# jwheo12/RustRayTrace

Measured on AMD Instinct MI355X. Metric: Mrays/sec + wall-clock for 1920×1080×512spp RTOW final scene, higher is better.
Workload: dtype f32; 1 GPU; C2 RTOW final scene (gpu/mod.rs generator, seed 0x5EED1234), 1920x1080x512spp, max_depth 100, 486 spheres; spp=512, max_depth=100, parallelism=whole frame on 1 GPU (the band split with one rank), no gather

## Files before the change

### include/rrt_hip.h

```cpp
#ifndef RRT_HIP_H
#define RRT_HIP_H

#include <stddef.h>
#include <stdint.h>

#ifdef __cplusplus
extern "C" {
#endif

#define RRT_ABI_VERSION 11u


typedef struct RrtCamera {
    float origin[4];
    float pixel00[4];
    float pixel_delta_u[4];
    float pixel_delta_v[4];
    float u[4];
    float v[4];
    float background[4];
    float params_f[4];
    uint32_t params_u[4];
} RrtCamera;

// ... 478 lines not shown
int32_t rrt_testing_launch_plan(const RrtLaunchPlanQuery *query, RrtLaunchPlan *plan);

int32_t rrt_testing_recip_check(uint64_t *mismatches);

int32_t rrt_testing_trig32_check(double *out);

int32_t rrt_testing_sqrt64_check(uint64_t *out);

enum RrtDeviceOp {
    RRT_OP_SIN = 0,
    RRT_OP_COS = 1,
    RRT_OP_LOG = 2,
    RRT_OP_ACOS = 3,
    RRT_OP_ATAN2 = 4,
    RRT_OP_DIV_A = 5,
    RRT_OP_DIV_CONST = 6,
    RRT_OP_FLOOR_I32 = 7,
    RRT_OP_CHECKER = 8,
    RRT_OP_PERLIN = 9,
    RRT_OP_VEC = 10,
    RRT_OP_QUAD = 11,
    RRT_OP_SPHERE = 12,
    RRT_OP_LIGHTS_PDF = 13,
    RRT_OP_LIGHTS_RANDOM = 14
};
int32_t rrt_testing_device_ops(uint32_t op, uint32_t n, const void *in, void *out, const void *aux);

int32_t rrt_testing_div_check(const float *a_values, uint32_t n_a, uint64_t *out);

enum RrtDeviceOp64 {
    RRT_OP_ACOS64 = 0,
    RRT_OP_ATAN2_64 = 1,
    RRT_OP_DIV_A64 = 2,
    RRT_OP_DIV_CONST64 = 3,
    RRT_OP_SQRT64 = 4,
    RRT_OP_AS_I32 = 5,
    RRT_OP_ATT64 = 6,
    RRT_OP_VEC64 = 7,
    RRT_OP_TEXEL64 = 8,
    RRT_OP_SPHERE64 = 9,
    RRT_OP_QUAD64 = 10,
    RRT_OP_CHECKER64 = 11
};
int32_t rrt_testing_device_ops64(uint32_t op, uint32_t n, const void *in, void *out, const void *aux);

#ifdef __cplusplus
}
// ... 3 lines not shown
```

### rustraytrace_amd/_lib.py

```python
from __future__ import annotations

import ctypes
import os
from ctypes import POINTER, c_char_p, c_double, c_float, c_int32, c_size_t, c_uint8, c_uint32, c_uint64, c_void_p

import numpy as np

PKG_DIR = os.path.dirname(os.path.abspath(__file__))
LIB_PATH = os.environ.get("RRT_LIB_PATH") or os.path.join(PKG_DIR, "librrt_hip.so")

CAMERA_DTYPE = np.dtype(
    [
        ("origin", "<f4", 4),
        ("pixel00", "<f4", 4),
        ("pixel_delta_u", "<f4", 4),
        ("pixel_delta_v", "<f4", 4),
        ("u", "<f4", 4),
        ("v", "<f4", 4),
        ("background", "<f4", 4),
        ("params_f", "<f4", 4),
        ("params_u", "<u4", 4),
    ]
)
SPHERE_DTYPE = np.dtype([("center_radius", "<f4", 4), ("material_index", "<u4"), ("_pad", "<u4", 3)])
# ... 129 lines not shown

class RrtSceneBuildStats(ctypes.Structure):
    _fields_ = [("builder", c_uint64), ("launches", c_uint64), ("blocking_reads", c_uint64), ("form", c_uint64),
                ("shape_attempts", c_uint64)]


BUILDERS = {"binned": 0, "lbvh": 1}


class RrtTreeCost(ctypes.Structure):
    _fields_ = [("sah", c_double), ("sah_at_build", c_double), ("refits_since_build", c_uint64)]


def refit_form(form: int) -> None:
    check(load().rrt_testing_refit_form(int(form)))

def lbvh_form(form: int) -> None:
    check(load().rrt_testing_lbvh_form(int(form)))

DEVICE_OPS = {
    "SIN": (0, 1, 1), "COS": (1, 1, 1), "LOG": (2, 1, 1), "ACOS": (3, 1, 1), "ATAN2": (4, 2, 1),
    "DIV_A": (5, 2, 4), "DIV_CONST": (6, 1, 4), "FLOOR_I32": (7, 1, 1), "CHECKER": (8, 4, 1),
    "PERLIN": (9, 3, 8), "VEC": (10, 9, 13), "QUAD": (11, 9, 2), "SPHERE": (12, 11, 13),
    "LIGHTS_PDF": (13, 6, 1), "LIGHTS_RANDOM": (14, 6, 4),
}

DEVICE_OPS64 = {
    "ACOS64": (0, 1, 1), "ATAN2_64": (1, 2, 1), "DIV_A64": (2, 2, 3), "DIV_CONST64": (3, 1, 4), "SQRT64": (4, 1, 1),
    "AS_I32": (5, 1, 1), "ATT64": (6, 2, 4), "VEC64": (7, 9, 11), "TEXEL64": (8, 5, 6), "SPHERE64": (9, 11, 6),
    "QUAD64": (10, 9, 2), "CHECKER64": (11, 4, 1),
}


class RrtTexture(ctypes.Structure):
    _fields_ = [("rgb8", POINTER(c_uint8)), ("width", c_int32), ("height", c_int32)]


PERLIN_DTYPE = np.dtype([("randvec", "<f4", (256, 4)), ("perm_x", "<u2", 256), ("perm_y", "<u2", 256),
                         ("perm_z", "<u2", 256), ("_pad", "<u2", 256)])


QUAD_DTYPE = np.dtype([("q", "<f4", 4), ("u", "<f4", 4), ("v", "<f4", 4), ("material_index", "<u4"),
                       ("_pad", "<u4", 3)])


LIGHT_DTYPE = np.dtype([("kind", "<u4"), ("_pad", "<u4", 3), ("a", "<f4", 4), ("u", "<f4", 4), ("v", "<f4", 4)])

# ... 326 lines not shown
```

### rustraytrace_amd/csrc/rrt_kernel.hip

```cpp
#include "rrt_internal.h"
#include "../../include/rrt_hip.h"

#include <algorithm>
#include <cstddef>
#include <cstdio>
#include <cstdlib>
#include <type_traits>

namespace rrt {
namespace {

#ifndef RRT_PHASE_TIMING
#define RRT_PHASE_TIMING 0
#endif
#ifndef RRT_DEBUG_NOREJECT
#define RRT_DEBUG_NOREJECT 0
#endif
#ifndef RRT_DEBUG_EXTRA_NODE_LOAD
#define RRT_DEBUG_EXTRA_NODE_LOAD 0
#endif
#ifndef RRT_PRIO_REFILL
#define RRT_PRIO_REFILL 2
#endif
#ifndef RRT_PRIO_NODE
// ... 160 lines not shown
__device__ __forceinline__ bool box_hit_ordered(float nx, float fx, float ny, float fy, float nz, float fz, V3 inv,
                                                V3 oi, float tmin, float tmax, float &tnear) {
    const float x0 = __builtin_fmaf(nx, inv.x, -oi.x), x1 = __builtin_fmaf(fx, inv.x, -oi.x);
    const float y0 = __builtin_fmaf(ny, inv.y, -oi.y), y1 = __builtin_fmaf(fy, inv.y, -oi.y);
    const float z0 = __builtin_fmaf(nz, inv.z, -oi.z), z1 = __builtin_fmaf(fz, inv.z, -oi.z);
    const float nr = __builtin_fmaxf(__builtin_fmaxf(x0, y0), __builtin_fmaxf(z0, tmin));
    const float fr = min_f32_raw(__builtin_fminf(__builtin_fminf(x1, y1), z1), tmax);
    tnear = nr;
    return nr < fr;
}


struct RayK {
    V3 inv;
    V3 oi;
    float a;
    float ra;
    uint32_t ox, oy, oz;
};

__device__ __forceinline__ float clamp_inv(float v) { return __builtin_fmaxf(__builtin_fminf(v, 0x1.0p64f), -0x1.0p64f); }
__device__ __forceinline__ float clamped_slope(float s) {
    return __builtin_fabsf(s) < 0x1.0p-126f ? __builtin_copysignf(0x1.0p64f, s) : clamp_inv(recip_rn(s));
}

#ifndef RRT_F16_ORDERED_MAX_CLASS
#define RRT_F16_ORDERED_MAX_CLASS 3
#endif
#ifndef RRT_B1U_WAVES
#define RRT_B1U_WAVES 8
#endif
#ifndef RRT_B1U_BLOCK
#define RRT_B1U_BLOCK 1024
#endif
#ifndef RRT_B1D_WAVES
#define RRT_B1D_WAVES 8
#endif
#ifndef RRT_B2_NF_WAVES
#define RRT_B2_NF_WAVES 6
#endif
#ifndef RRT_B2_MEDIA_GLOBAL_WAVES
#define RRT_B2_MEDIA_GLOBAL_WAVES 0
#endif
__device__ __forceinline__ float refine_ra(float a) {
    const float r0 = __builtin_amdgcn_rcpf(a);
    const float e = __builtin_fmaf(-a, r0, 1.0f);
    return (a >= 0x1.0p-64f && a <= 0x1.0p64f) ? __builtin_fmaf(e, r0, r0) : 0.0f;
}
template <bool kLdsNodes = true, bool kHoldRa = true>
__device__ __forceinline__ RayK ray_consts(V3 o, V3 d) {
    RayK r;
    r.inv = v3(clamped_slope(d.x), clamped_slope(d.y), clamped_slope(d.z));
    r.oi = v3(o.x * r.inv.x, o.y * r.inv.y, o.z * r.inv.z);
    if (kLdsNodes) {
        r.ox = r.inv.x < 0.0f ? 4u : 0u;
        r.oy = r.inv.y < 0.0f ? 16u : 12u;
        r.oz = r.inv.z < 0.0f ? 28u : 24u;
    } else {
        r.ox = (r.inv.x < 0.0f ? 16u : 0u) | (r.inv.y < 0.0f ? 16u << 5 : 0u) | (r.inv.z < 0.0f ? 16u << 10 : 0u);
        r.oy = r.oz = 0u;
    }
    r.a = dot(d, d);
    r.ra = kHoldRa ? refine_ra(r.a) : 0.0f;
    return r;
}

__device__ __forceinline__ float div_by_a(float n, const RayK &rk) {
    const float q0 = n * rk.ra;
    const float m = __builtin_fabsf(q0);
    const bool outside = !(m >= 0x1.0p-30f && m < __builtin_inff());
    const float e0 = __builtin_fmaf(-rk.a, q0, n);
    const float q1 = __builtin_fmaf(e0, rk.ra, q0);
    const float e1 = __builtin_fmaf(-rk.a, q1, n);
    float q = __builtin_fmaf(e1, rk.ra, q1);
    if (__ballot(outside) != 0) {
        float nn = n;
        asm volatile("" : "+v"(nn));
        if (outside) q = nn / rk.a;
    }
    return q;
}

constexpr int kBook1Untextured = -1;
constexpr int kBook1Diffuse = -2;
template <int kBook2>
struct Prims {
    const float4 *cr;
    const float4 *mo;
    float time;
    const GQuad *qd;
    const GMedium *md;
    uint32_t n_quads;
    uint64_t seg;
    const GPerlin *perlin;
    static constexpr bool kHasQuads = kBook2 >= 2;
    static constexpr bool kHasMedia = kBook2 >= 3;
// ... 187 lines not shown
    if constexpr (RRT_PHASE_TIMING == 3) cnt.d2 += 1;
    const float sq = sqrt_rn_disc(disc);
    float root = div_by_a(h - sq, rk);
    uint64_t lt = __ballot(root < closest);
    asm volatile("" : "+v"(root));
    const bool below = !(0.001f < root);
    if (__builtin_expect(__ballot(below) != 0, 0)) {
        float hh = h;
        asm volatile("" : "+v"(hh));
        if (below) root = div_by_a(hh + sq, rk);
        lt = __ballot(0.001f < root) & __ballot(root < closest);
    }
    const bool accept = __builtin_amdgcn_inverse_ballot_w64(lt);
    closest = accept ? root : closest;
    hit_prim = accept ? i : hit_prim;
}

template <bool kCount, class PR>
__device__ __forceinline__ void test_range(const PR &prim_cr, int first, int count, V3 o, V3 d, const RayK &rk,
                                           int skip, float &closest, int &hit_prim, Counters &cnt) {
    if (kCount) cnt.spheres += (uint32_t)count;
    const bool trim = (uint32_t)(skip - first) < (uint32_t)count;
    const int n = count - (trim ? 1 : 0);
    const int gap = trim ? skip : 0x7fffffff;
    for (int k = 0; k < n; ++k) {
        const int i = first + k + (first + k >= gap ? 1 : 0);
        if constexpr (RRT_PHASE_TIMING == 3) {
            cnt.d0 += wave_slot();
            cnt.d1 += 1;
        }
        const float4 cr = prim_cr.cr[i];
        float4 m = cr;
        if constexpr (!PR::kR2) m = prim_cr.mo[i];
        test_prim(prim_cr, cr, m, i, o, d, rk, closest, hit_prim, cnt);
    }
}


struct Trav {
    float closest;
    int hit_prim;
    int node;
    uint32_t sp;
};

__device__ __forceinline__ void trav_begin(Trav &t, int root, uint32_t sp0) {
    t.closest = __builtin_inff();
    t.hit_prim = -1;
    t.node = root;
// ... 135 lines not shown
    cswap(0, 2);
    cswap(1, 3);
    cswap(1, 2);
    const float kInf = __builtin_inff();
    if (key[3] < kInf) { stack.store(t.sp, idx[3]); ++t.sp; }
    if (key[2] < kInf) { stack.store(t.sp, idx[2]); ++t.sp; }
    if (key[1] < kInf) { stack.store(t.sp, idx[1]); ++t.sp; }
    if (key[0] < kInf) {
        t.node = idx[0];
        return false;
    }
    if (t.sp == 0) {
        t.node = -1;
        return true;
    }
    --t.sp;
    t.node = stack.load(t.sp);
    return false;
}

struct PathState {
    V3 o, d, T;
    RngState rng;
    uint32_t k;
    float time;
    int skip;
};

__device__ __forceinline__ int exit_skip(bool is_quad, bool is_medium, bool front, V3 dir, V3 nrm, int prim) {
    if (is_medium) return -1;
    if (is_quad) return prim;
    return ((dot(dir, nrm) > 0.0f) == front) ? prim : -1;
}

template <bool kStrat>
__device__ __forceinline__ void camera_ray(const KParams &P, uint32_t x, uint32_t y, uint32_t s, PathState &ps,
                                           Counters &cnt) {
    const auto &C = *kernarg_params();
    float ox, oy;
    if constexpr (kStrat) {
        const uint32_t sj = fast_div(s, P.fd_sqrt_spp), si = s - sj * P.sqrt_spp;
        ox = (((float)si + rnd(ps.rng)) * P.recip_sqrt_spp) - 0.5f;
        oy = (((float)sj + rnd(ps.rng)) * P.recip_sqrt_spp) - 0.5f;
    } else {
        ox = __builtin_fmaf((float)(rng_next(ps.rng) >> 8), 0x1.0p-24f, -0.5f);
        oy = __builtin_fmaf((float)(rng_next(ps.rng) >> 8), 0x1.0p-24f, -0.5f);
    }
    const float fi = (float)x + ox;
    const float fj = (float)y + oy;
    const V3 sample = v3(C.p00[0] + C.du[0] * fi + C.dv[0] * fj,
                         C.p00[1] + C.du[1] * fi + C.dv[1] * fj,
                         C.p00[2] + C.du[2] * fi + C.dv[2] * fj);
    V3 origin = v3(C.center[0], C.center[1], C.center[2]);
    if (C.defocus_radius > 0.0f) {
        float px, py;
        for (;;) {
            if constexpr (RRT_PHASE_TIMING == 7) cnt.d2 += wave_slot();
            px = rnd_pm1(ps.rng);
            py = rnd_pm1(ps.rng);
            if (__builtin_fmaf(py, py, px * px) < 1.0f) break;
        }
        origin = v3(C.center[0] + C.disk_u[0] * px + C.disk_v[0] * py,
                    C.center[1] + C.disk_u[1] * px + C.disk_v[1] * py,
                    C.center[2] + C.disk_u[2] * px + C.disk_v[2] * py);
    }
    ps.time = 0.0f;
    if (C.flags & 0x1u) ps.time = rnd(ps.rng);
    ps.skip = -1;
    ps.o = origin;
    ps.d = sub(sample, origin);
    ps.T = v3(1.0f, 1.0f, 1.0f);
    ps.k = 0;
}

__device__ __forceinline__ RngState path_rng(const KParams &P, uint32_t x, uint32_t y, uint32_t s) {
    const uint64_t key = pixel_key(P, x, y);
    return rng_seed(splitmix64(key + s), key);
}

__device__ __forceinline__ float rrt_sinf(float xx) {
    float x = xx;
    float sign = 1.0f;
    if (x < 0.0f) { sign = -1.0f; x = -x; }
    if (x > 16777215.0f) return 0.0f;
    if (!(x == x)) return xx;
    int j = (int)(1.27323954473516f * x);
    float y = (float)j;
    if (j & 1) { j += 1; y += 1.0f; }
    j &= 7;
    if (j > 3) { sign = -sign; j -= 4; }
    if (x > 8192.0f) x = x - y * 0.7853981633974483096f;
    else x = ((x - y * 0.78515625f) - y * 2.4187564849853515625e-4f) - y * 3.77489497744594108e-8f;
    const float z = x * x;
    if (j == 1 || j == 2) {
        y = ((2.443315711809948e-5f * z - 1.388731625493765e-3f) * z + 4.166664568298827e-2f) * z * z;
// ... 126 lines not shown
        cnt.d0 += wave_slot();
        cnt.d1 += 1;
    }
    if constexpr (RRT_PHASE_TIMING == 9) cnt.d2 += wave_slot();
    if (prim < 0) {
        if constexpr (RRT_PHASE_TIMING == 6) {
            cnt.d1 += wave_slot();
            cnt.d2 += 1;
        }
        V3 bg;
        if (P.bg_mode == 1u) {
            bg = v3(P.background[0], P.background[1], P.background[2]);
        } else {
            const V3 ud = unit(ps.d);
            const float a = 0.5f * (ud.y + 1.0f);
            bg = v3((1.0f - a) * 1.0f + a * 0.5f, (1.0f - a) * 1.0f + a * 0.7f, (1.0f - a) * 1.0f + a * 1.0f);
        }
        sum = add(sum, mul(ps.T, bg));
        return true;
    }
    float4 qn;
    const float4 cr = prims.at(prim, qn);
    const V3 p = v3(__builtin_fmaf(ps.d.x, t, ps.o.x), __builtin_fmaf(ps.d.y, t, ps.o.y), __builtin_fmaf(ps.d.z, t, ps.o.z));
    V3 outward;
    bool is_quad = false, is_medium = false;
    if (PR::kHasQuads && cr.w < 0.0f) {
        const int j = (int)(-cr.w) - 1;
        if (PR::kHasMedia && j >= (int)prims.n_quads) {
            is_medium = true;
            outward = v3(1.0f, 0.0f, 0.0f);
        } else {
            is_quad = true;
            outward = v3(qn.x, qn.y, qn.z);
        }
    } else {
        const float inv_r = PR::kR2 ? __int_as_float(mtl[prim].b.w) : qn.w;
        outward = v3((p.x - cr.x) * inv_r, (p.y - cr.y) * inv_r, (p.z - cr.z) * inv_r);
    }
    const bool front = dot(ps.d, outward) < 0.0f;
    const V3 nrm = front ? outward : v3(-outward.x, -outward.y, -outward.z);
    const GMaterial m = mtl[prim];
    const int kind = m.b.x;
    V3 att;
    V3 dir;
    if (kind == 4) {
        sum = add(sum, mul(ps.T, v3(m.a.x, m.a.y, m.a.z)));
// ... 12 lines not shown
#define RRT_DEBUG_TEXEL_FIXED 0
#endif
            const float theta = RRT_DEBUG_TEXEL_FIXED ? 1.0f + outward.y * 0x1.0p-30f : rrt_acosf(-outward.y);
            const float phi = RRT_DEBUG_TEXEL_FIXED ? 2.0f + outward.x * 0x1.0p-30f : rrt_atan2f(-outward.z, outward.x) + kPi;
            att = texel(P, m.b.z, div_by_const(phi, 2.0f * kPi), div_by_const(theta, kPi));
        } else if (kBook2 > 0 && kind == 5) {
            att = checker_even(m.a.w, p) ? v3(m.a.x, m.a.y, m.a.z)
                                         : v3(__int_as_float(m.b.y), __int_as_float(m.b.z), __int_as_float(m.b.w));
        } else if (kBook2 > 0 && kNoise && kind == 6) {
            if constexpr (RRT_PHASE_TIMING == 9) {
                cnt.d0 += wave_slot();
                cnt.d1 += 1;
            }
            const float g = noise_at(P, prims.perlin, m.b.z, m.a.w, p);
            att = v3(g, g, g);
        } else {
            att = v3(m.a.x, m.a.y, m.a.z);
        }
    } else if (kind == 1) {
        if constexpr (RRT_PHASE_TIMING == 5) cnt.d2 += wave_slot();
        if constexpr (RRT_PHASE_TIMING == 6) cnt.d0 += 1;
        const V3 refl = unit(reflect(ps.d, nrm));
        dir = add(refl, muls(r, m.a.w));
        if (!(dot(dir, nrm) > 0.0f)) return true;
        att = v3(m.a.x, m.a.y, m.a.z);
    } else {
        if constexpr (RRT_PHASE_TIMING == 5) {
            cnt.d0 += wave_slot();
            cnt.d1 += 1;
        }
        float ri, r0;
        dielectric_ri_r0(m, front, ri, r0);
        const V3 ud = unit(ps.d);
        float c = -dot(ud, nrm);
        c = (c < 1.0f) ? c : 1.0f;
        const float sn = sqrt_rn_big(1.0f - c * c);
        const bool cannot = ri * sn > 1.0f;
        if (cannot || reflectance_r0(c, r0) > rnd(ps.rng)) dir = reflect(ud, nrm);
        else dir = refract(ud, nrm, ri);
        att = v3(1.0f, 1.0f, 1.0f);
    }
    if (ps.k >= 5u) {
        float pr = att.x;
        if (att.y > pr) pr = att.y;
        if (att.z > pr) pr = att.z;
        if (pr < 0.05f) pr = 0.05f;
        if (pr > 0.95f) pr = 0.95f;
        if (rnd(ps.rng) > pr) return true;
        float inv_pr;
        if (kBook2 == kBook1Untextured) inv_pr = kind == 2 ? 1.0f / 0.95f : __int_as_float(m.b.y);
        else inv_pr = recip_rn(pr);
        ps.T = muls(mul(ps.T, att), inv_pr);
    } else {
        ps.T = mul(ps.T, att);
    }
    ps.o = p;
    ps.d = dir;
    ps.k++;
    ps.skip = exit_skip(is_quad, is_medium, front, dir, nrm, prim);
    return false;
}

__device__ __forceinline__ V3 onb_transform(V3 n, V3 a) {
    const V3 w = unit(n);
    const V3 ax = (__builtin_fabsf(w.x) > 0.9f) ? v3(0.0f, 1.0f, 0.0f) : v3(1.0f, 0.0f, 0.0f);
    const V3 v = unit(cross(w, ax));
    const V3 u = cross(w, v);
    return v3(a.x * u.x + a.y * v.x + a.z * w.x, a.x * u.y + a.y * v.y + a.z * w.y, a.x * u.z + a.y * v.z + a.z * w.z);
}

__device__ __forceinline__ bool sphere_root(float4 c, V3 o, V3 d, float tmin) {
    const V3 oc = v3(c.x - o.x, c.y - o.y, c.z - o.z);
    const float a = dot(d, d);
    const float h = dot(d, oc);
    const float cc = dot(oc, oc) - c.w * c.w;
    const float disc = __builtin_fmaf(h, h, -(a * cc));
    if (disc < 0.0f) return false;
    const float sq = __builtin_sqrtf(disc);
    const float inf = __builtin_inff();
    float root = (h - sq) / a;
    if (!(tmin < root && root < inf)) {
        root = (h + sq) / a;
// ... 37 lines not shown
        const float r2 = rnd(rng);
        const V3 p = v3(a.x + r2 * g.v.x, a.y + r2 * g.v.y, a.z + r2 * g.v.z);
        return sub(p, o);
    }
    const V3 dir = v3(L.sphere.x - o.x, L.sphere.y - o.y, L.sphere.z - o.z);
    const float d2 = dot(dir, dir);
    const float r1 = rnd(rng), r2 = rnd(rng);
    const float z = 1.0f + r2 * (__builtin_sqrtf(1.0f - L.sphere.w * L.sphere.w / d2) - 1.0f);
    const float phi = (2.0f * kPi) * r1;
    const float sxy = __builtin_sqrtf(1.0f - z * z);
    return onb_transform(dir, v3(rrt_cosf(phi) * sxy, rrt_sinf(phi) * sxy, z));
}

template <bool kNoise, typename C, class PR>
__device__ __forceinline__ bool shade_b3(const KParams &P, const PR &prims, const GMaterial *mtl, PathState &ps,
                                         float t, int prim, V3 &sum, C &cnt) {
    if (prim < 0) {
        sum = add(sum, mul(ps.T, v3(P.background[0], P.background[1], P.background[2])));
        return true;
    }
    float4 qn;
    const float4 cr = prims.at(prim, qn);
    const V3 p = v3(__builtin_fmaf(ps.d.x, t, ps.o.x), __builtin_fmaf(ps.d.y, t, ps.o.y), __builtin_fmaf(ps.d.z, t, ps.o.z));
    V3 outward;
    bool is_quad = false, is_medium = false;
    if (cr.w < 0.0f) {
        const int j = (int)(-cr.w) - 1;
        if (j >= (int)prims.n_quads) {
            is_medium = true;
            outward = v3(1.0f, 0.0f, 0.0f);
        } else {
            is_quad = true;
            outward = v3(qn.x, qn.y, qn.z);
        }
    } else {
        const float inv_r = qn.w;
        outward = v3((p.x - cr.x) * inv_r, (p.y - cr.y) * inv_r, (p.z - cr.z) * inv_r);
    }
    const bool front = (cr.w < 0.0f && (int)(-cr.w) - 1 >= (int)prims.n_quads) ? true : dot(ps.d, outward) < 0.0f;
    const V3 nrm = front ? outward : v3(-outward.x, -outward.y, -outward.z);
    const GMaterial m = mtl[prim];
    const int kind = m.b.x;
    if (kind == 4) {
        if (front) sum = add(sum, mul(ps.T, v3(m.a.x, m.a.y, m.a.z)));
        return true;
    }
    V3 att, dir;
    if (kind == 1 || kind == 2) {
        if (kind == 1) {
            const V3 r = random_unit_vector(ps.rng, cnt);
            const V3 refl = unit(reflect(ps.d, nrm));
            dir = add(refl, muls(r, m.a.w));
            att = v3(m.a.x, m.a.y, m.a.z);
        } else {
            float ri, r0;
            dielectric_ri_r0(m, front, ri, r0);
            const V3 ud = unit(ps.d);
            float c = -dot(ud, nrm);
            c = (c < 1.0f) ? c : 1.0f;
            const float sn = sqrt_rn_big(1.0f - c * c);
            const bool cannot = ri * sn > 1.0f;
            if (cannot || reflectance_r0(c, r0) > rnd(ps.rng)) dir = reflect(ud, nrm);
            else dir = refract(ud, nrm, ri);
            att = v3(1.0f, 1.0f, 1.0f);
        }
        if (ps.k >= 5u) {
            float pr = att.x;
            if (att.y > pr) pr = att.y;
            if (att.z > pr) pr = att.z;
            if (pr < 0.05f) pr = 0.05f;
            if (pr > 0.95f) pr = 0.95f;
            if (rnd(ps.rng) > pr) return true;
            ps.T = muls(mul(ps.T, att), 1.0f / pr);
        } else {
            ps.T = mul(ps.T, att);
        }
        ps.o = p;
        ps.d = dir;
        ps.k++;
        ps.skip = exit_skip(is_quad, is_medium, front, dir, nrm, prim);
        return false;
    }
    if (kind == 3) {
        const float theta = rrt_acosf(-outward.y);
        const float phi = rrt_atan2f(-outward.z, outward.x) + kPi;
        att = texel(P, m.b.z, div_by_const(phi, 2.0f * kPi), div_by_const(theta, kPi));
    } else if (kind == 5) {
        att = checker_even(m.a.w, p) ? v3(m.a.x, m.a.y, m.a.z)
                                     : v3(__int_as_float(m.b.y), __int_as_float(m.b.z), __int_as_float(m.b.w));
    } else if (kNoise && kind == 6) {
        const float g = noise_at(P, prims.perlin, m.b.z, m.a.w, p);
        att = v3(g, g, g);
    } else {
        att = v3(m.a.x, m.a.y, m.a.z);
    }
    float rr = 1.0f;
    if (ps.k >= 5u) {
        rr = att.x;
        if (att.y > rr) rr = att.y;
        if (att.z > rr) rr = att.z;
        if (rr < 0.05f) rr = 0.05f;
        if (rr > 0.95f) rr = 0.95f;
        if (rr < 1.0f && rnd(ps.rng) > rr) return true;
    }
    const bool iso = kind == 7;
    const float inv4pi = 1.0f / (4.0f * kPi);
    if (rnd(ps.rng) < 0.5f) {
        dir = lights_random(P, p, ps.rng);
    } else if (iso) {
        dir = random_unit_vector(ps.rng, cnt);
    } else {
        const float r1 = rnd(ps.rng), r2 = rnd(ps.rng);
        const float phi = (2.0f * kPi) * r1;
        const float sr2 = __builtin_sqrtf(r2);
        dir = onb_transform(nrm, v3(rrt_cosf(phi) * sr2, rrt_sinf(phi) * sr2, __builtin_sqrtf(1.0f - r2)));
    }
    float mat_pdf;
    if (iso) {
        mat_pdf = inv4pi;
    } else {
        const float cosine = dot(unit(dir), unit(nrm));
        mat_pdf = cosine <= 0.0f ? 0.0f : cosine / kPi;
    }
    const float pdf = 0.5f * lights_pdf(P, p, dir) + 0.5f * mat_pdf;
    if (pdf <= 0.0f) return true;
    float spdf;
    if (iso) {
        spdf = inv4pi;
    } else {
        const float cosine = dot(nrm, unit(dir));
        spdf = cosine < 0.0f ? 0.0f : cosine / kPi;
    }
    ps.T = mul(ps.T, muls(muls(att, spdf), 1.0f / (pdf * rr)));
    ps.o = p;
    ps.d = dir;
    ps.k++;
    ps.skip = exit_skip(is_quad, is_medium, front, dir, nrm, prim);
    return false;
}

template <int kBook2, bool kNoise, typename C, class PR>
__device__ __forceinline__ bool shade_any(const KParams &P, const PR &prims, const GMaterial *mtl, PathState &ps,
                                          float t, int prim, V3 &sum, C &cnt) {
    if constexpr (kBook2 == 4) return shade_b3<kNoise>(P, prims, mtl, ps, t, prim, sum, cnt);
    else return shade<kBook2, kNoise>(P, prims, mtl, ps, t, prim, sum, cnt);
}

__device__ __forceinline__ void trace_segment(uint32_t xy, uint32_t s, const PathState &ps, float t, int prim) {
#ifdef RRT_TRACE_X
    if ((xy & 0xffffu) == RRT_TRACE_X && (xy >> 16) == RRT_TRACE_Y && s == RRT_TRACE_S)
        printf("K k=%u o=(%a %a %a) d=(%a %a %a) t=%a prim=%d T=(%a %a %a) rng=%llx\n", ps.k, ps.o.x, ps.o.y, ps.o.z,
               ps.d.x, ps.d.y, ps.d.z, t, prim, ps.T.x, ps.T.y, ps.T.z, (unsigned long long)rng_key(ps.rng));
#endif
}

template <bool kLds, bool kCount, typename StackT, bool kWide, int kBook2, int kBlk, bool kNoise>
__device__ __forceinline__ void render_body(const KParams &P) {
    extern __shared__ uint4 lds_dyn[];
    uint32_t stack16 = 0;
    [[maybe_unused]] const uint32_t node_base = kLds && !kWide ? lds_addr(lds_dyn) : 0u;
    using Node = typename std::conditional<kWide, GNode4, typename std::conditional<kLds, GNode, GNodeH>::type>::type;
    const Node *nodes = reinterpret_cast<const Node *>(P.nodes);
    const float4 *prims = P.prim_cr;
    const GMaterial *mtl = P.prim_mtl;
    const float4 *motion = P.prim_motion;
    if constexpr (kLds) {
        uint4 *dst = lds_dyn;
        const uint4 *src_n = reinterpret_cast<const uint4 *>(P.nodes);
        constexpr uint32_t kNode16 = (uint32_t)(sizeof(Node) / 16);
        const uint32_t nn = P.n_nodes * kNode16;
        for (uint32_t i = threadIdx.x; i < nn; i += kBlk) {
            uint4 v = src_n[i];
            if constexpr (!kWide) {
                static_assert(offsetof(GNode, link) == sizeof(GNode) - 8, "GNode links end the record");
// ... 22 lines not shown
        if constexpr (kBook2 > 0) motion = reinterpret_cast<const float4 *>(dst + nn + P.n_prims + nm);
    }
    const GPerlin *perlin = P.perlin;
    if constexpr (kBook2 > 0) {
        if (P.perlin_in_lds) {
            size_t off16 = stack16;
            if constexpr (!kLds) off16 = (P.stack_depth * kBlk * sizeof(StackT) + 15u) / 16u;
            uint4 *dst = lds_dyn + off16;
            const uint4 *src = reinterpret_cast<const uint4 *>(P.perlin);
            const uint32_t n16 = P.n_perlin * (uint32_t)(sizeof(GPerlin) / 16);
            for (uint32_t i = threadIdx.x; i < n16; i += kBlk) dst[i] = src[i];
            __syncthreads();
            perlin = reinterpret_cast<const GPerlin *>(dst);
            if constexpr (kLds) stack16 += n16;
        }
    }
    StackT *lds_stack = reinterpret_cast<StackT *>(lds_dyn + stack16);
    LdsStack<StackT, kBlk> stack;
    stack.init(lds_stack, threadIdx.x);

    const uint32_t lane = threadIdx.x & 63u;
    Counters cnt = {0, 0, 0, 0, 0, 0};
    uint32_t w_rays = 0, w_paths = 0;
    uint32_t has = 0;
    bool q_open = true;
    uint32_t xy = 0, s = 0, s_hi = 0;
    uint64_t pkey = 0;
    V3 sum = v3(0.0f, 0.0f, 0.0f);
    PathState ps;
    Trav tr;
    tr.node = -1;
    uint32_t need_ray = 0;
    uint32_t pool_base = (blockIdx.x & (kQueues - 1u)) * 64u, pool_left = 0;
    [[maybe_unused]] uint64_t ph0 = 0, ph1 = 0, ph2 = 0, tp = 0;
    for (;;) {
        if constexpr (RRT_PHASE_TIMING == 1) tp = __builtin_amdgcn_s_memtime();
        if constexpr (RRT_PHASE_TIMING == 2) ph2++;
        __builtin_amdgcn_s_setprio(RRT_PRIO_REFILL);
        uint64_t idle = __ballot(!has);
        if (idle != 0 && pool_left == 0 && q_open) {
            const uint32_t xq = (pool_base >> 6) & (kQueues - 1u);
            uint32_t k = 0;
            if (lane == 0) k = atomicAdd(P.unit_counter + 32u * xq, 1u);
            const uint32_t base = ((uint32_t)__builtin_amdgcn_readlane((int)k, 0) * kQueues + xq) * 64u;
            if (base >= P.n_units) {
                q_open = false;
            } else {
                pool_base = base;
                pool_left = min(64u, P.n_units - base);
            }
        }
        if (idle != 0 && pool_left != 0) {
            const uint32_t n = min((uint32_t)__popcll(idle), pool_left);
            const uint32_t r = __builtin_amdgcn_mbcnt_hi((uint32_t)(idle >> 32), __builtin_amdgcn_mbcnt_lo((uint32_t)idle, 0u));
            if (!has && r < n) {
                const uint32_t u = pool_base + r;
                {
                    const auto &Q = *kernarg_params();
                    const uint32_t lit = u & 63u;
                    const uint32_t tc = u >> 6;
                    uint32_t t, chunk;
                    if (u < Q.n_big_units) {
                        t = fast_div(tc, fdiv(Q.fd_pass_big));
                        chunk = Q.chunk_begin + (tc - t * Q.pass_big);
                    } else {
                        const uint32_t ns = Q.pass_n - Q.pass_big, tc2 = tc - (Q.n_big_units >> 6);
                        t = fast_div(tc2, fdiv(Q.fd_pass_tail));
                        chunk = Q.chunk_begin + Q.pass_big + (tc2 - t * ns);
                    }
                    const uint32_t ty = fast_div(t, fdiv(Q.fd_tiles_x));
                    const uint32_t x = (t - ty * Q.tiles_x) * kTileW + (lit % kTileW);
                    const uint32_t ly = ty * kTileH + (lit / kTileW);
                    if (x < Q.width && ly < Q.tile_rows) {
                        const uint32_t band = fast_div(ly, fdiv(Q.fd_band_rows));
                        const uint32_t slot = (band & 1u) ? Q.n_ranks - 1u - Q.rank : Q.rank;
                        const uint32_t y = (band * Q.n_ranks + slot) * Q.band_rows + (ly - band * Q.band_rows);
                        xy = x | (y << 16);
                        s = Q.sample_begin + chunk_first(Q, chunk);
                        s_hi = min(s + (chunk < Q.n_big ? Q.chunk : Q.chunk_small), Q.sample_end);
                        sum = v3(0.0f, 0.0f, 0.0f);
                        pkey = pixel_key(Q, x, y);
                        ps.rng = path_rng_k(pkey, s);
                        camera_ray<kBook2 == 4>(P, x, y, s, ps, cnt);
                        need_ray = 1;
                        has = 1;
                    }
                }
            }
            pool_base += n;
            pool_left -= n;
        }
        if (__ballot(has) == 0) break;

        uint32_t seg_done = 0;
        uint32_t started = 0;
        if (has && need_ray) {
            if (ps.k >= P.max_depth) {
                seg_done = 1;
            } else {
                trav_begin(tr, kWide ? 0 : (int)node_base, kWide ? 0u : stack.bottom);
                need_ray = 0;
                started = 1;
            }
        }
        w_rays += (uint32_t)__popcll(__ballot(started));
        const uint32_t live = (uint32_t)__popcll(__ballot(has));
        const uint32_t min_active = (live * P.trav_frac) >> 8;
        if constexpr (RRT_PHASE_TIMING == 1) {
            const uint64_t t = __builtin_amdgcn_s_memtime();
            ph0 += t - tp;
            tp = t;
        }
        RayK rk;
        constexpr bool kOrd16 = !kLds && !kWide && kBook2 <= RRT_F16_ORDERED_MAX_CLASS;
        constexpr bool kHoldRa = !(kOrd16 && kBook2 == 3);
        if (tr.node >= 0) rk = ray_consts<!kOrd16, kHoldRa>(ps.o, ps.d);
        const Prims<kBook2> pr{prims, motion, ps.time, P.quads, P.media, P.n_quads, rng_key(ps.rng) ^ ((uint64_t)ps.k << 32), perlin};
        if constexpr (kWide) {
            for (;;) {
                if constexpr (RRT_PHASE_TIMING == 2) {
                    ph0 += 64;
                    ph1 += (uint64_t)__popcll(__ballot(tr.node >= 0));
                }
                if (tr.node >= 0) trav_step4<kCount>(nodes, pr, stack, ps.o, ps.d, rk, ps.skip, tr, cnt);
                if ((uint32_t)__popcll(__ballot(tr.node >= 0)) <= min_active) break;
            }
        } else {
            const uint32_t leaf_min = (live * P.leaf_frac) >> 8;
            __builtin_amdgcn_s_setprio(RRT_PRIO_NODE);
            Leaves lv = 0;
            uint64_t step = __ballot(tr.node >= 0);
            for (;;) {
                if constexpr (RRT_PHASE_TIMING == 2) {
                    ph0 += 64;
                    ph1 += (uint64_t)__popcll(__ballot(tr.node >= 0 && lv == 0));
                }
                if constexpr (RRT_PHASE_TIMING == 8) {
                    const bool stepping = tr.node >= 0 && lv == 0;
                    const uint64_t sm = __ballot(stepping);
                    const int n0 = __builtin_amdgcn_readfirstlane(stepping ? tr.node : 0x7fffffff);
// ... 11 lines not shown
                const uint64_t nm = __ballot(tr.node >= 0);
                step = nm & ~pm;
                const int32_t waiting = __popcll(pm), stepping = __popcll(step);
                const int32_t leave = waiting + stepping - (int32_t)min_active - 1;
                const int32_t batch = ((int32_t)leaf_min - waiting) | leave | (stepping - 1);
                if (batch < 0) {
                    __builtin_amdgcn_s_setprio(RRT_PRIO_LEAF);
                    if (__builtin_amdgcn_inverse_ballot_w64(pm)) {
                        trav_leaves<kCount, kHoldRa>(pr, lv, ps.o, ps.d, rk, ps.skip, tr, cnt);
                        lv = 0;
                    }
                    step = nm;
                    __builtin_amdgcn_s_setprio(RRT_PRIO_NODE);
                }
                if (leave < 0) break;
            }
        }
        __builtin_amdgcn_s_setprio(RRT_PRIO_SHADE);
        if constexpr (RRT_PHASE_TIMING == 1) {
            const uint64_t t = __builtin_amdgcn_s_memtime();
            ph1 += t - tp;
            tp = t;
        }
        const bool shading = has && !need_ray && tr.node < 0;
        if (shading) {
            need_ray = 1;
            const Prims<kBook2> spr{prims, motion, ps.time, P.quads, P.media, P.n_quads, rng_key(ps.rng) ^ ((uint64_t)ps.k << 32), perlin};
            if constexpr (Prims<kBook2>::kHasMedia) {
                if (!kHoldRa) rk.ra = refine_ra(rk.a);
                for (uint32_t u = P.n_prims - P.n_unbounded; u < P.n_prims; ++u) {
                    if (kCount) cnt.spheres++;
                    const int m = (int)(-prims[u].w) - 1 - (int)P.n_quads;
                    float tm;
                    if (medium_hit(spr, m, ps.o, ps.d, rk, tr.closest, tm)) {
                        tr.closest = tm;
                        tr.hit_prim = (int)u;
                    }
                }
            }
            trace_segment(xy, s, ps, tr.closest, tr.hit_prim);
            seg_done = shade_any<kBook2, kNoise>(P, spr, mtl, ps, tr.closest, tr.hit_prim, sum, cnt) ? 1u : 0u;
        }
        w_paths += (uint32_t)__popcll(__ballot(seg_done));
        if (seg_done) {
            ++s;
            const uint32_t x = xy & 0xffffu, y = xy >> 16;
            if (s < s_hi) {
                ps.rng = path_rng_k(pkey, s);
                if constexpr (RRT_PHASE_TIMING == 7) {
                    cnt.d0 += wave_slot();
                    cnt.d1 += 1;
                }
                camera_ray<kBook2 == 4>(P, x, y, s, ps, cnt);
            } else {
                const auto &Q = *kernarg_params();
                const uint32_t rel = s_hi - 1u - Q.sample_begin;
                const uint32_t nbs = Q.n_big * Q.chunk;
                const uint32_t chunk =
                    rel < nbs ? fast_div(rel, fdiv(Q.fd_chunk)) : Q.n_big + fast_div(rel - nbs, fdiv(Q.fd_chunk_small));
                const uint32_t gb = fast_div(y, fdiv(Q.fd_band_rows));
                const uint32_t ly = fast_div(gb, fdiv(Q.fd_n_ranks)) * Q.band_rows + (y - gb * Q.band_rows);
                const size_t px = (size_t)ly * Q.width + x;
                const float4 out = make_float4(sum.x, sum.y, sum.z, (float)(s_hi - (Q.sample_begin + chunk_first(Q, chunk))));
                if (Q.n_chunks == 1) Q.accum[px] = out;
                else Q.partial[(size_t)(chunk - Q.chunk_begin) * ((size_t)Q.tile_rows * Q.width) + px] = F3{sum.x, sum.y, sum.z};
                has = 0;
            }
        }
        if constexpr (RRT_PHASE_TIMING == 1) ph2 += __builtin_amdgcn_s_memtime() - tp;
    }
    if constexpr (((RRT_PHASE_TIMING >= 3 && RRT_PHASE_TIMING <= 7) || RRT_PHASE_TIMING == 9) && !kCount) {
        ph0 = wave_sum_u32(cnt.d0);
        ph1 = wave_sum_u32(cnt.d1);
        ph2 = wave_sum_u32(cnt.d2);
    }
    if constexpr (RRT_PHASE_TIMING != 0 && !kCount) {
        if (lane == 0) {
            atomicAdd(&P.counters[2], (unsigned long long)ph0);
            atomicAdd(&P.counters[3], (unsigned long long)ph1);
            atomicAdd(&P.counters[4], (unsigned long long)ph2);
        }
    }
    const uint32_t r = w_rays;
    const uint32_t pa = w_paths;
    uint32_t nv = 0, bt = 0, st = 0;
    if (kCount) {
        nv = wave_sum_u32(cnt.nodes);
        bt = wave_sum_u32(cnt.boxes);
        st = wave_sum_u32(cnt.spheres);
    }
    if (lane == 0) {
        if (r) atomicAdd(&P.counters[0], (unsigned long long)r);
        if (pa) atomicAdd(&P.counters[1], (unsigned long long)pa);
        if (kCount) {
            atomicAdd(&P.counters[2], (unsigned long long)nv);
            atomicAdd(&P.counters[3], (unsigned long long)bt);
            atomicAdd(&P.counters[4], (unsigned long long)st);
        }
    }
}

template <bool kLds, bool kCount, typename StackT, bool kWide, int kWaves, int kBook2, int kBlk, bool kNoise>
__global__ __launch_bounds__(kBlk, kWaves) void rrt_render(KParams P) {
    render_body<kLds, kCount, StackT, kWide, kBook2, kBlk, kNoise>(P);
}

__global__ __launch_bounds__(256) void rrt_combine_chunks(const F3 *__restrict__ partial, float4 *__restrict__ accum,
                                                          uint32_t n_pixels, uint32_t n_chunks, uint32_t first,
                                                          float count) {
    const uint32_t p = blockIdx.x * 256u + threadIdx.x;
    if (p >= n_pixels) return;
    float4 acc;
    if (first) {
        const F3 v = partial[p];
        acc = make_float4(v.x, v.y, v.z, 0.0f);
    } else {
        acc = accum[p];
    }
    for (uint32_t c = first ? 1u : 0u; c < n_chunks; ++c) {
        const F3 v = partial[(size_t)c * n_pixels + p];
// ... 372 lines not shown
            const V3 v = ld3(x), nn = ld3(x + 3);
            st3(r, unit(v));
            st3(r + 3, reflect(v, nn));
            st3(r + 6, refract(v, nn, x[6]));
            r[9] = __float_as_uint(reflectance_r0(x[7], x[8]));
            st3(r + 10, onb_transform(nn, v));
            break;
        }
        case RRT_OP_QUAD: {
            const uint32_t j = (uint32_t)x[8];
            float t = 0.0f;
            const bool hit = j < n_aux && quad_hit(reinterpret_cast<const GQuad *>(aux)[j], ld3(x), ld3(x + 3), x[6], x[7], t);
            r[0] = hit ? 1u : 0u;
            r[1] = __float_as_uint(hit ? t : 0.0f);
            break;
        }
        case RRT_OP_SPHERE: {
            const V3 o = ld3(x), d = ld3(x + 3);
            const float rad = x[9] < 0.0f ? 0.0f : x[9];
            const RayK rk = ray_consts(o, d);
            sphere_ops<0>(make_float4(x[6], x[7], x[8], rad * rad), o, d, rk, x[10], r);
            sphere_ops<1>(make_float4(x[6], x[7], x[8], rad), o, d, rk, x[10], r + 6);
            r[12] = sphere_root(make_float4(x[6], x[7], x[8], rad), o, d, 0.001f) ? 1u : 0u;
            break;
        }
        case RRT_OP_LIGHTS_PDF: r[0] = __float_as_uint(lights_pdf(LP, ld3(x), ld3(x + 3))); break;
        case RRT_OP_LIGHTS_RANDOM: {
            KParams Q = LP;
            Q.seed = __float_as_uint(x[3]);
            RngState rng = path_rng(Q, __float_as_uint(x[4]), 0u, __float_as_uint(x[5]));
            RngState replay = rng;
            st3(r, lights_random(LP, ld3(x), rng));
            uint32_t draws = 0;
            while (draws < 16u && !(replay.a == rng.a && replay.b == rng.b && replay.c == rng.c && replay.d == rng.d)) {
                rng_next(replay);
                ++draws;
            }
            r[3] = draws;
            break;
        }
        default: break;
        }
    }
}

__global__ __launch_bounds__(256) void rrt_div_check(const float *__restrict__ a_values, uint32_t n_a,
// ... 36 lines not shown
        if (s && __lane_id() == 0) atomicAdd(&out[i], (unsigned long long)s);
    }
}
}

hipError_t launch_recip_check(unsigned long long *d_out, hipStream_t stream) {
    hipLaunchKernelGGL(rrt_recip_check, dim3(16384), dim3(256), 0, stream, d_out);
    return hipGetLastError();
}

void device_op_columns(uint32_t op, uint32_t &cols_in, uint32_t &cols_out) {
    switch (op) {
    case RRT_OP_SIN: case RRT_OP_COS: case RRT_OP_LOG: case RRT_OP_ACOS: case RRT_OP_FLOOR_I32: cols_in = 1, cols_out = 1; break;
    case RRT_OP_ATAN2: cols_in = 2, cols_out = 1; break;
    case RRT_OP_DIV_A: cols_in = 2, cols_out = 4; break;
    case RRT_OP_DIV_CONST: cols_in = 1, cols_out = 4; break;
    case RRT_OP_CHECKER: cols_in = 4, cols_out = 1; break;
    case RRT_OP_PERLIN: cols_in = 3, cols_out = 8; break;
    case RRT_OP_VEC: cols_in = 9, cols_out = 13; break;
    case RRT_OP_QUAD: cols_in = 9, cols_out = 2; break;
    case RRT_OP_SPHERE: cols_in = 11, cols_out = 13; break;
    case RRT_OP_LIGHTS_PDF: cols_in = 6, cols_out = 1; break;
    case RRT_OP_LIGHTS_RANDOM: cols_in = 6, cols_out = 4; break;
    default: cols_in = cols_out = 0; break;
    }
}

hipError_t launch_device_ops(uint32_t op, uint32_t n, const float *d_in, uint32_t *d_out, const void *d_aux,
                             uint32_t n_aux, float scale, hipStream_t stream) {
    uint32_t cin = 0, cout = 0;
    device_op_columns(op, cin, cout);
    if (cin == 0 || n == 0) return hipErrorInvalidValue;
    const uint32_t blocks = std::min((n + 255u) / 256u, 8192u);
    hipLaunchKernelGGL(rrt_device_ops, dim3(blocks), dim3(256), 0, stream, op, n, cin, cout, d_in, d_out, d_aux, n_aux, scale);
    return hipGetLastError();
}

hipError_t launch_div_check(const float *d_a, uint32_t n_a, unsigned long long *d_out, hipStream_t stream) {
    hipLaunchKernelGGL(rrt_div_check, dim3(16384), dim3(256), 0, stream, d_a, n_a, d_out);
    return hipGetLastError();
}

}
```

Before: 38270 Mrays/s.

## Pack path state flags, add fast slope reciprocal path, trim register pressure

```diff
diff --git a/include/rrt_hip.h b/include/rrt_hip.h
--- a/include/rrt_hip.h
+++ b/include/rrt_hip.h
@@ -524,7 +524,8 @@
     RRT_OP_QUAD = 11,
     RRT_OP_SPHERE = 12,
     RRT_OP_LIGHTS_PDF = 13,
-    RRT_OP_LIGHTS_RANDOM = 14
+    RRT_OP_LIGHTS_RANDOM = 14,
+    RRT_OP_SLOPES = 15
 };
 int32_t rrt_testing_device_ops(uint32_t op, uint32_t n, const void *in, void *out, const void *aux);
 
diff --git a/rustraytrace_amd/_lib.py b/rustraytrace_amd/_lib.py
--- a/rustraytrace_amd/_lib.py
+++ b/rustraytrace_amd/_lib.py
@@ -175,7 +175,7 @@
     "SIN": (0, 1, 1), "COS": (1, 1, 1), "LOG": (2, 1, 1), "ACOS": (3, 1, 1), "ATAN2": (4, 2, 1),
     "DIV_A": (5, 2, 4), "DIV_CONST": (6, 1, 4), "FLOOR_I32": (7, 1, 1), "CHECKER": (8, 4, 1),
     "PERLIN": (9, 3, 8), "VEC": (10, 9, 13), "QUAD": (11, 9, 2), "SPHERE": (12, 11, 13),
-    "LIGHTS_PDF": (13, 6, 1), "LIGHTS_RANDOM": (14, 6, 4),
+    "LIGHTS_PDF": (13, 6, 1), "LIGHTS_RANDOM": (14, 6, 4), "SLOPES": (15, 6, 13),
 }
 
 DEVICE_OPS64 = {
diff --git a/rustraytrace_amd/csrc/rrt_kernel.hip b/rustraytrace_amd/csrc/rrt_kernel.hip
--- a/rustraytrace_amd/csrc/rrt_kernel.hip
+++ b/rustraytrace_amd/csrc/rrt_kernel.hip
@@ -206,6 +206,23 @@
 __device__ __forceinline__ float clamp_inv(float v) { return __builtin_fmaxf(__builtin_fminf(v, 0x1.0p64f), -0x1.0p64f); }
 __device__ __forceinline__ float clamped_slope(float s) {
     return __builtin_fabsf(s) < 0x1.0p-126f ? __builtin_copysignf(0x1.0p64f, s) : clamp_inv(recip_rn(s));
+}
+
+__device__ __forceinline__ float slope_normal(float s) {
+    const float r = __builtin_amdgcn_rcpf(s);
+    return clamp_inv(__builtin_fmaf(__builtin_fmaf(-s, r, 1.0f), r, r));
+}
+__device__ __forceinline__ V3 clamped_slopes(V3 d) {
+    constexpr int kNotNormal = 0x2f7;
+    const bool outside = __builtin_amdgcn_classf(d.x, kNotNormal) | __builtin_amdgcn_classf(d.y, kNotNormal) |
+                         __builtin_amdgcn_classf(d.z, kNotNormal);
+    V3 inv = v3(slope_normal(d.x), slope_normal(d.y), slope_normal(d.z));
+    if (__ballot(outside) != 0) {
+        V3 c = d;
+        asm volatile("" : "+v"(c.x), "+v"(c.y), "+v"(c.z));
+        if (outside) inv = v3(clamped_slope(c.x), clamped_slope(c.y), clamped_slope(c.z));
+    }
+    return inv;
 }
 
 #ifndef RRT_F16_ORDERED_MAX_CLASS
@@ -234,7 +251,7 @@
 template <bool kLdsNodes = true, bool kHoldRa = true>
 __device__ __forceinline__ RayK ray_consts(V3 o, V3 d) {
     RayK r;
-    r.inv = v3(clamped_slope(d.x), clamped_slope(d.y), clamped_slope(d.z));
+    r.inv = clamped_slopes(d);
     r.oi = v3(o.x * r.inv.x, o.y * r.inv.y, o.z * r.inv.z);
     if (kLdsNodes) {
         r.ox = r.inv.x < 0.0f ? 4u : 0u;
@@ -253,9 +270,9 @@
     const float q0 = n * rk.ra;
     const float m = __builtin_fabsf(q0);
     const bool outside = !(m >= 0x1.0p-30f && m < __builtin_inff());
-    const float e0 = __builtin_fmaf(-rk.a, q0, n);
+    const float e0 = __builtin_fmaf(rk.a, -q0, n);
     const float q1 = __builtin_fmaf(e0, rk.ra, q0);
-    const float e1 = __builtin_fmaf(-rk.a, q1, n);
+    const float e1 = __builtin_fmaf(rk.a, -q1, n);
     float q = __builtin_fmaf(e1, rk.ra, q1);
     if (__ballot(outside) != 0) {
         float nn = n;
@@ -489,9 +506,9 @@
     if (kCount) cnt.spheres += (uint32_t)count;
     const bool trim = (uint32_t)(skip - first) < (uint32_t)count;
     const int n = count - (trim ? 1 : 0);
-    const int gap = trim ? skip : 0x7fffffff;
+    const uint32_t gap = trim ? (uint32_t)skip : 0xffffffffu;
     for (int k = 0; k < n; ++k) {
-        const int i = first + k + (first + k >= gap ? 1 : 0);
+        const int i = first + k + ((uint32_t)(first + k) >= gap ? 1 : 0);
         if constexpr (RRT_PHASE_TIMING == 3) {
             cnt.d0 += wave_slot();
             cnt.d1 += 1;
@@ -673,10 +690,13 @@
 struct PathState {
     V3 o, d, T;
     RngState rng;
-    uint32_t k;
+    uint32_t st;
     float time;
     int skip;
 };
+
+constexpr uint32_t kStHas = 1u, kStNeedRay = 2u, kStBounce = 4u;
+constexpr uint32_t kStRouletteFrom = 5u * kStBounce;
 
 __device__ __forceinline__ int exit_skip(bool is_quad, bool is_medium, bool front, V3 dir, V3 nrm, int prim) {
     if (is_medium) return -1;
@@ -721,7 +741,7 @@
     ps.o = origin;
     ps.d = sub(sample, origin);
     ps.T = v3(1.0f, 1.0f, 1.0f);
-    ps.k = 0;
+    ps.st = kStHas | kStNeedRay;
 }
 
 __device__ __forceinline__ RngState path_rng(const KParams &P, uint32_t x, uint32_t y, uint32_t s) {
@@ -894,6 +914,7 @@
     float4 qn;
     const float4 cr = prims.at(prim, qn);
     const V3 p = v3(__builtin_fmaf(ps.d.x, t, ps.o.x), __builtin_fmaf(ps.d.y, t, ps.o.y), __builtin_fmaf(ps.d.z, t, ps.o.z));
+    ps.o = p;
     V3 outward;
     bool is_quad = false, is_medium = false;
     if (PR::kHasQuads && cr.w < 0.0f) {
@@ -952,7 +973,10 @@
         if constexpr (RRT_PHASE_TIMING == 6) cnt.d0 += 1;
         const V3 refl = unit(reflect(ps.d, nrm));
         dir = add(refl, muls(r, m.a.w));
-        if (!(dot(dir, nrm) > 0.0f)) return true;
+        if (!(dot(dir, nrm) > 0.0f)) {
+            ps.d = dir;
+            return true;
+        }
         att = v3(m.a.x, m.a.y, m.a.z);
     } else {
         if constexpr (RRT_PHASE_TIMING == 5) {
@@ -970,7 +994,10 @@
         else dir = refract(ud, nrm, ri);
         att = v3(1.0f, 1.0f, 1.0f);
     }
-    if (ps.k >= 5u) {
+    ps.d = dir;
+    ps.skip = exit_skip(is_quad, is_medium, front, dir, nrm, prim);
+    ps.T = mul(ps.T, att);
+    if (ps.st >= kStRouletteFrom) {
         float pr = att.x;
         if (att.y > pr) pr = att.y;
         if (att.z > pr) pr = att.z;
@@ -980,14 +1007,9 @@
         float inv_pr;
         if (kBook2 == kBook1Untextured) inv_pr = kind == 2 ? 1.0f / 0.95f : __int_as_float(m.b.y);
         else inv_pr = recip_rn(pr);
-        ps.T = muls(mul(ps.T, att), inv_pr);
-    } else {
-        ps.T = mul(ps.T, att);
-    }
-    ps.o = p;
-    ps.d = dir;
-    ps.k++;
-    ps.skip = exit_skip(is_quad, is_medium, front, dir, nrm, prim);
+        ps.T = muls(ps.T, inv_pr);
+    }
+    ps.st += kStBounce;
     return false;
 }
 
@@ -1071,6 +1093,7 @@
     float4 qn;
     const float4 cr = prims.at(prim, qn);
     const V3 p = v3(__builtin_fmaf(ps.d.x, t, ps.o.x), __builtin_fmaf(ps.d.y, t, ps.o.y), __builtin_fmaf(ps.d.z, t, ps.o.z));
+    ps.o = p;
     V3 outward;
     bool is_quad = false, is_medium = false;
     if (cr.w < 0.0f) {
@@ -1113,7 +1136,8 @@
             else dir = refract(ud, nrm, ri);
             att = v3(1.0f, 1.0f, 1.0f);
         }
-        if (ps.k >= 5u) {
+        ps.d = dir;
+        if (ps.st >= kStRouletteFrom) {
             float pr = att.x;
             if (att.y > pr) pr = att.y;
             if (att.z > pr) pr = att.z;
@@ -1124,12 +1148,11 @@
         } else {
             ps.T = mul(ps.T, att);
         }
-        ps.o = p;
-        ps.d = dir;
-        ps.k++;
+        ps.st += kStBounce;
         ps.skip = exit_skip(is_quad, is_medium, front, dir, nrm, prim);
         return false;
     }
+    ps.d = nrm;
     if (kind == 3) {
         const float theta = rrt_acosf(-outward.y);
         const float phi = rrt_atan2f(-outward.z, outward.x) + kPi;
@@ -1144,7 +1167,7 @@
         att = v3(m.a.x, m.a.y, m.a.z);
     }
     float rr = 1.0f;
-    if (ps.k >= 5u) {
+    if (ps.st >= kStRouletteFrom) {
         rr = att.x;
         if (att.y > rr) rr = att.y;
         if (att.z > rr) rr = att.z;
@@ -1181,9 +1204,8 @@
         spdf = cosine < 0.0f ? 0.0f : cosine / kPi;
     }
     ps.T = mul(ps.T, muls(muls(att, spdf), 1.0f / (pdf * rr)));
-    ps.o = p;
     ps.d = dir;
-    ps.k++;
+    ps.st += kStBounce;
     ps.skip = exit_skip(is_quad, is_medium, front, dir, nrm, prim);
     return false;
 }
@@ -1198,7 +1220,7 @@
 __device__ __forceinline__ void trace_segment(uint32_t xy, uint32_t s, const PathState &ps, float t, int prim) {
 #ifdef RRT_TRACE_X
     if ((xy & 0xffffu) == RRT_TRACE_X && (xy >> 16) == RRT_TRACE_Y && s == RRT_TRACE_S)
-        printf("K k=%u o=(%a %a %a) d=(%a %a %a) t=%a prim=%d T=(%a %a %a) rng=%llx\n", ps.k, ps.o.x, ps.o.y, ps.o.z,
+        printf("K k=%u o=(%a %a %a) d=(%a %a %a) t=%a prim=%d T=(%a %a %a) rng=%llx\n", ps.st >> 2, ps.o.x, ps.o.y, ps.o.z,
                ps.d.x, ps.d.y, ps.d.z, t, prim, ps.T.x, ps.T.y, ps.T.z, (unsigned long long)rng_key(ps.rng));
 #endif
 }
@@ -1267,7 +1289,6 @@
     const uint32_t lane = threadIdx.x & 63u;
     Counters cnt = {0, 0, 0, 0, 0, 0};
     uint32_t w_rays = 0, w_paths = 0;
-    uint32_t has = 0;
     bool q_open = true;
     uint32_t xy = 0, s = 0, s_hi = 0;
     uint64_t pkey = 0;
@@ -1275,14 +1296,14 @@
     PathState ps;
     Trav tr;
     tr.node = -1;
-    uint32_t need_ray = 0;
+    ps.st = 0;
     uint32_t pool_base = (blockIdx.x & (kQueues - 1u)) * 64u, pool_left = 0;
     [[maybe_unused]] uint64_t ph0 = 0, ph1 = 0, ph2 = 0, tp = 0;
     for (;;) {
         if constexpr (RRT_PHASE_TIMING == 1) tp = __builtin_amdgcn_s_memtime();
         if constexpr (RRT_PHASE_TIMING == 2) ph2++;
         __builtin_amdgcn_s_setprio(RRT_PRIO_REFILL);
-        uint64_t idle = __ballot(!has);
+        uint64_t idle = __ballot(ps.st == 0);
         if (idle != 0 && pool_left == 0 && q_open) {
             const uint32_t xq = (pool_base >> 6) & (kQueues - 1u);
             uint32_t k = 0;
@@ -1298,7 +1319,7 @@
         if (idle != 0 && pool_left != 0) {
             const uint32_t n = min((uint32_t)__popcll(idle), pool_left);
             const uint32_t r = __builtin_amdgcn_mbcnt_hi((uint32_t)(idle >> 32), __builtin_amdgcn_mbcnt_lo((uint32_t)idle, 0u));
-            if (!has && r < n) {
+            if (ps.st == 0 && r < n) {
                 const uint32_t u = pool_base + r;
                 {
                     const auto &Q = *kernarg_params();
@@ -1327,29 +1348,27 @@
                         pkey = pixel_key(Q, x, y);
                         ps.rng = path_rng_k(pkey, s);
                         camera_ray<kBook2 == 4>(P, x, y, s, ps, cnt);
-                        need_ray = 1;
-                        has = 1;
                     }
                 }
             }
             pool_base += n;
             pool_left -= n;
         }
-        if (__ballot(has) == 0) break;
+        if (__ballot(ps.st != 0) == 0) break;
 
         uint32_t seg_done = 0;
         uint32_t started = 0;
-        if (has && need_ray) {
-            if (ps.k >= P.max_depth) {
+        if ((ps.st & (kStHas | kStNeedRay)) == (kStHas | kStNeedRay)) {
+            if ((ps.st >> 2) >= P.max_depth) {
                 seg_done = 1;
             } else {
                 trav_begin(tr, kWide ? 0 : (int)node_base, kWide ? 0u : stack.bottom);
-                need_ray = 0;
+                ps.st &= ~kStNeedRay;
                 started = 1;
             }
         }
         w_rays += (uint32_t)__popcll(__ballot(started));
-        const uint32_t live = (uint32_t)__popcll(__ballot(has));
+        const uint32_t live = (uint32_t)__popcll(__ballot(ps.st != 0));
         const uint32_t min_active = (live * P.trav_frac) >> 8;
         if constexpr (RRT_PHASE_TIMING == 1) {
             const uint64_t t = __builtin_amdgcn_s_memtime();
@@ -1360,7 +1379,7 @@
         constexpr bool kOrd16 = !kLds && !kWide && kBook2 <= RRT_F16_ORDERED_MAX_CLASS;
         constexpr bool kHoldRa = !(kOrd16 && kBook2 == 3);
         if (tr.node >= 0) rk = ray_consts<!kOrd16, kHoldRa>(ps.o, ps.d);
-        const Prims<kBook2> pr{prims, motion, ps.time, P.quads, P.media, P.n_quads, rng_key(ps.rng) ^ ((uint64_t)ps.k << 32), perlin};
+        const Prims<kBook2> pr{prims, motion, ps.time, P.quads, P.media, P.n_quads, rng_key(ps.rng) ^ ((uint64_t)(ps.st >> 2) << 32), perlin};
         if constexpr (kWide) {
             for (;;) {
                 if constexpr (RRT_PHASE_TIMING == 2) {
@@ -1418,10 +1437,10 @@
             ph1 += t - tp;
             tp = t;
         }
-        const bool shading = has && !need_ray && tr.node < 0;
+        const bool shading = (ps.st & (kStHas | kStNeedRay)) == kStHas && tr.node < 0;
         if (shading) {
-            need_ray = 1;
-            const Prims<kBook2> spr{prims, motion, ps.time, P.quads, P.media, P.n_quads, rng_key(ps.rng) ^ ((uint64_t)ps.k << 32), perlin};
+            ps.st |= kStNeedRay;
+            const Prims<kBook2> spr{prims, motion, ps.time, P.quads, P.media, P.n_quads, rng_key(ps.rng) ^ ((uint64_t)(ps.st >> 2) << 32), perlin};
             if constexpr (Prims<kBook2>::kHasMedia) {
                 if (!kHoldRa) rk.ra = refine_ra(rk.a);
                 for (uint32_t u = P.n_prims - P.n_unbounded; u < P.n_prims; ++u) {
@@ -1460,7 +1479,7 @@
                 const float4 out = make_float4(sum.x, sum.y, sum.z, (float)(s_hi - (Q.sample_begin + chunk_first(Q, chunk))));
                 if (Q.n_chunks == 1) Q.accum[px] = out;
                 else Q.partial[(size_t)(chunk - Q.chunk_begin) * ((size_t)Q.tile_rows * Q.width) + px] = F3{sum.x, sum.y, sum.z};
-                has = 0;
+                ps.st = 0;
             }
         }
         if constexpr (RRT_PHASE_TIMING == 1) ph2 += __builtin_amdgcn_s_memtime() - tp;
@@ -1486,12 +1505,13 @@
         st = wave_sum_u32(cnt.spheres);
     }
     if (lane == 0) {
-        if (r) atomicAdd(&P.counters[0], (unsigned long long)r);
-        if (pa) atomicAdd(&P.counters[1], (unsigned long long)pa);
+        unsigned long long *counters = kernarg_params()->counters;
+        if (r) atomicAdd(&counters[0], (unsigned long long)r);
+        if (pa) atomicAdd(&counters[1], (unsigned long long)pa);
         if (kCount) {
-            atomicAdd(&P.counters[2], (unsigned long long)nv);
-            atomicAdd(&P.counters[3], (unsigned long long)bt);
-            atomicAdd(&P.counters[4], (unsigned long long)st);
+            atomicAdd(&counters[2], (unsigned long long)nv);
+            atomicAdd(&counters[3], (unsigned long long)bt);
+            atomicAdd(&counters[4], (unsigned long long)st);
         }
     }
 }
@@ -1910,6 +1930,18 @@
             sphere_ops<0>(make_float4(x[6], x[7], x[8], rad * rad), o, d, rk, x[10], r);
             sphere_ops<1>(make_float4(x[6], x[7], x[8], rad), o, d, rk, x[10], r + 6);
             r[12] = sphere_root(make_float4(x[6], x[7], x[8], rad), o, d, 0.001f) ? 1u : 0u;
+            break;
+        }
+        case RRT_OP_SLOPES: {
+            const V3 o = ld3(x), d = ld3(x + 3);
+            const RayK rk = ray_consts(o, d);
+            st3(r, rk.inv);
+            st3(r + 3, rk.oi);
+            r[6] = rk.ox;
+            r[7] = rk.oy;
+            r[8] = rk.oz;
+            st3(r + 9, v3(clamped_slope(d.x), clamped_slope(d.y), clamped_slope(d.z)));
+            r[12] = ray_consts<false>(o, d).ox;
             break;
         }
         case RRT_OP_LIGHTS_PDF: r[0] = __float_as_uint(lights_pdf(LP, ld3(x), ld3(x + 3))); break;
@@ -1992,6 +2024,7 @@
     case RRT_OP_SPHERE: cols_in = 11, cols_out = 13; break;
     case RRT_OP_LIGHTS_PDF: cols_in = 6, cols_out = 1; break;
     case RRT_OP_LIGHTS_RANDOM: cols_in = 6, cols_out = 4; break;
+    case RRT_OP_SLOPES: cols_in = 6, cols_out = 13; break;
     default: cols_in = cols_out = 0; break;
     }
 }
```

Measured after the change: 39440 Mrays/s, median of 6. 1.03x the previous value.
